# gkaissis/PriMIA

Measured on AMD Instinct MI355X. Metric: images_per_sec, higher is better.
Workload: dtype bf16; 1 GPU; ResNet-18 federated-client training step (fwd+loss+bwd+SGD), batch 256/client, 3x224x224, 1 client per GPU; batch_per_client=256, clients=1, sync_every_n_batch=3, dp_sgd=False

## Files before the change

### primia_amd/build.py

```python
import concurrent.futures
import os
import shutil
import subprocess
import sys

HERE = os.path.dirname(os.path.abspath(__file__))
CSRC = os.path.join(HERE, "csrc")
OBJ = os.path.join(CSRC, "_build")
ISA = os.path.join(OBJ, "isa")
LIB = os.path.join(HERE, "libprimia_hip.so")
ARCH = "gfx950"
FLAGS = ["-O3", "-std=c++17", "-fPIC", f"--offload-arch={ARCH}", "-Wno-unused-result"]


def source_digest(files=None):
    import hashlib

    names = sorted(f for f in os.listdir(CSRC) if f.endswith((".hip", ".h"))) if files is None else sorted(files)
    paths = [os.path.join(CSRC, f) for f in names]
    if files is None:
        paths.append(os.path.join(HERE, "..", "include", "primia_hip.h"))
    h = hashlib.sha256()
    for q in paths:
        h.update(os.path.basename(q).encode() + b"\0")
        import re

        text = re.sub(r"/\*.*?\*/", "", open(q, "r", encoding="utf-8", errors="replace").read(), flags=re.S)
        for line in text.splitlines():
            code = line.split("//", 1)[0].rstrip()
            if code:
                h.update(code.encode() + b"\n")
    return h.hexdigest()


def _hipcc():
    for c in ("/opt/rocm/bin/hipcc", "hipcc"):
        if os.path.isabs(c) and os.path.exists(c):
            return c
    return "hipcc"


def _newer(src, dst, deps=()):
    if not os.path.exists(dst):
        return True
    t = os.path.getmtime(dst)
    return any(os.path.getmtime(p) > t for p in (src, *deps))


def build(force=False, verbose=True):
    os.makedirs(OBJ, exist_ok=True)
    headers = [os.path.join(CSRC, f) for f in os.listdir(CSRC) if f.endswith(".h")]
    headers.append(os.path.join(HERE, "..", "include", "primia_hip.h"))
    sources = sorted(f for f in os.listdir(CSRC) if f.endswith(".hip"))
    jobs = []
    for f in sources:
        src = os.path.join(CSRC, f)
        obj = os.path.join(OBJ, f[:-4] + ".o")
        if force or _newer(src, obj, headers) or not os.path.exists(os.path.join(ISA, f[:-4] + ".s")):
            jobs.append((src, obj))

    def compile_one(job):
        src, obj = job
        name = os.path.basename(src)[:-4]
        tmp = os.path.join(OBJ, "tmp_" + name)
        shutil.rmtree(tmp, ignore_errors=True)
        os.makedirs(tmp)
        cmd = [_hipcc(), *FLAGS, "-save-temps=obj", "-c", src, "-o", os.path.join(tmp, name + ".o")]
        r = subprocess.run(cmd, capture_output=True, text=True)
        if r.returncode == 0:
            os.makedirs(ISA, exist_ok=True)
            os.replace(os.path.join(tmp, f"{name}-hip-amdgcn-amd-amdhsa-{ARCH}.s"), os.path.join(ISA, name + ".s"))
            os.replace(os.path.join(tmp, name + ".o"), obj)
        shutil.rmtree(tmp, ignore_errors=True)
        return src, r.returncode, r.stdout + r.stderr

    if jobs:
        with concurrent.futures.ThreadPoolExecutor(max_workers=min(6, len(jobs))) as ex:
            for src, rc, out in ex.map(compile_one, jobs):
                if verbose:
                    print(f"[primia build] {os.path.basename(src)}: {'ok' if rc == 0 else 'FAILED'}")
                if rc != 0:
                    raise RuntimeError(f"hipcc failed for {src}:\n{out}")
    objs = [os.path.join(OBJ, f[:-4] + ".o") for f in sources]
    if jobs or force or not os.path.exists(LIB):
        cmd = [_hipcc(), "-shared", "-fPIC", f"--offload-arch={ARCH}", "-o", LIB, *objs]
        r = subprocess.run(cmd, capture_output=True, text=True)
        if r.returncode != 0:
            raise RuntimeError("link failed:\n" + r.stdout + r.stderr)
        if verbose:
            print(f"[primia build] linked {LIB}")
    return LIB


PROBE_LIB = os.path.join(HERE, "..", "tools", "micro", "libprimia_probe.so")
PROBE_SOURCES = ("conv3x3_c64.hip", "conv_s2lh.hip", "options.hip")


def build_probe(extra_flags=()):
    build(verbose=False)
    objs = []
    for f in sorted(x for x in os.listdir(CSRC) if x.endswith(".hip")):
        if f in PROBE_SOURCES:
            os.makedirs(os.path.join(OBJ, "probe"), exist_ok=True)
            obj = os.path.join(OBJ, "probe", f[:-4] + ".o")
            cmd = [_hipcc(), *FLAGS, "-DPRIMIA_PROBE=1", *extra_flags, "-c", os.path.join(CSRC, f), "-o", obj]
            r = subprocess.run(cmd, capture_output=True, text=True)
            if r.returncode != 0:
                raise RuntimeError(f"hipcc failed for {f} (probe):\n{r.stdout}{r.stderr}")
        else:
            obj = os.path.join(OBJ, f[:-4] + ".o")
        objs.append(obj)
    r = subprocess.run([_hipcc(), "-shared", "-fPIC", f"--offload-arch={ARCH}", "-o", PROBE_LIB, *objs],
                       capture_output=True, text=True)
    if r.returncode != 0:
        raise RuntimeError("link failed:\n" + r.stdout + r.stderr)
    print(f"[primia build] linked {os.path.normpath(PROBE_LIB)}")
    return PROBE_LIB


if __name__ == "__main__":
    if "--probe" in sys.argv:
        build_probe()
    else:
        build(force="--force" in sys.argv)
```

### primia_amd/csrc/options.h

```cpp
#pragma once

namespace primia {

#define PRIMIA_OPTIONS(X)                                                                                              \
    X(lh2, 1)                                        \
    X(lh2_bm, 0)                                      \
    X(lh4, 1)                \
    X(c64_blocks, 512)                                         \
    X(c64_dbg, 0)                      \
    X(c64_stages, 4)                                                      \
    X(s2lh, 1)               \
    X(s2lh_dbg, 0)

enum OptId : int {
#define PRIMIA_OPT_ENUM(name, def) kOpt_##name,
    PRIMIA_OPTIONS(PRIMIA_OPT_ENUM)
#undef PRIMIA_OPT_ENUM
        kOptCount
};

extern int g_options[kOptCount];

inline int opt(OptId id) { return __atomic_load_n(&g_options[id], __ATOMIC_RELAXED); }

}

#define PRIMIA_OPT(name) (::primia::opt(::primia::kOpt_##name))
```

### primia_amd/csrc/options.hip

```cpp
#include <string.h>

#include <atomic>

#include "common.h"
#include "options.h"

#ifndef PRIMIA_PROBE
#define PRIMIA_PROBE 0
#endif

namespace primia {

int g_options[kOptCount] = {
#define PRIMIA_OPT_DEF(name, def) def,
    PRIMIA_OPTIONS(PRIMIA_OPT_DEF)
#undef PRIMIA_OPT_DEF
};

static const char* const kOptNames[kOptCount] = {
#define PRIMIA_OPT_NAME(name, def) #name,
    PRIMIA_OPTIONS(PRIMIA_OPT_NAME)
#undef PRIMIA_OPT_NAME
};

static const int kOptDefaults[kOptCount] = {
#define PRIMIA_OPT_DEF(name, def) def,
    PRIMIA_OPTIONS(PRIMIA_OPT_DEF)
#undef PRIMIA_OPT_DEF
};

static std::atomic<int64_t> g_options_epoch{0};

static int find_option(const char* name) {
    if (!name) return -1;
    for (int i = 0; i < kOptCount; ++i)
        if (!strcmp(name, kOptNames[i])) return i;
    return -1;
}

}

using namespace primia;

extern "C" {

int primia_set_option(const char* name, int value) {
    const int i = find_option(name);
    if (i < 0) return PRIMIA_ERR_ARG;
#if !PRIMIA_PROBE
    if ((i == kOpt_c64_dbg || i == kOpt_s2lh_dbg) && value != 0) return PRIMIA_ERR_UNSUPPORTED;
#endif
    if (__atomic_exchange_n(&g_options[i], value, __ATOMIC_RELAXED) != value)
        g_options_epoch.fetch_add(1, std::memory_order_release);
    return PRIMIA_OK;
}

int64_t primia_options_epoch(void) { return g_options_epoch.load(std::memory_order_acquire); }

int primia_get_option(const char* name, int* value) {
    const int i = find_option(name);
    if (i < 0 || !value) return PRIMIA_ERR_ARG;
    *value = __atomic_load_n(&g_options[i], __ATOMIC_RELAXED);
    return PRIMIA_OK;
}

int primia_reset_options(void) {
    bool moved = false;
    for (int i = 0; i < kOptCount; ++i) moved |= __atomic_exchange_n(&g_options[i], kOptDefaults[i], __ATOMIC_RELAXED) != kOptDefaults[i];
    if (moved) g_options_epoch.fetch_add(1, std::memory_order_release);
    return PRIMIA_OK;
}

int primia_option_count(void) { return kOptCount; }

int primia_option_name(int index, char* buf, int buf_len) {
    if (index < 0 || index >= kOptCount || !buf || buf_len <= (int)strlen(kOptNames[index])) return PRIMIA_ERR_ARG;
    strcpy(buf, kOptNames[index]);
    return PRIMIA_OK;
}

}
```

### primia_amd/csrc/stem_bwd_fused.hip

```cpp
#include <stdlib.h>

#include "conv_wgrad.h"

namespace primia {

__device__ __attribute__((aligned(16))) const unsigned char kStemFusedZeroPage[16] = {0};

__device__ __forceinline__ void sbf_dma16(const void* g, unsigned lds_addr) {
    asm volatile("s_mov_b32 m0, %1\n\ts_nop 0\n\tglobal_load_lds_dwordx4 %0, off" ::"v"(g), "s"(lds_addr) : "memory");
}

typedef int sbf_i32x4 __attribute__((ext_vector_type(4)));

__device__ __forceinline__ void sbf_bdma16(unsigned voff, sbf_i32x4 rsrc, unsigned lds_addr) {
    asm volatile("s_mov_b32 m0, %2\n\ts_nop 0\n\tbuffer_load_dwordx4 %0, %1, 0 offen lds"
                 ::"v"(voff), "s"(rsrc), "s"(lds_addr) : "memory");
}

__device__ __forceinline__ sbf_i32x4 sbf_rsrc(const void* base, long bytes) {
    const unsigned long long a = (unsigned long long)base;
    sbf_i32x4 r;
    r[0] = (int)(unsigned)a;
    r[1] = (int)(unsigned)(a >> 32) & 0xffff;
    r[2] = (int)(unsigned)(bytes > 0xfffffff0L ? 0xfffffff0L : bytes);
    r[3] = 0x00020000;
#pragma unroll
    for (int j = 0; j < 4; ++j) r[j] = __builtin_amdgcn_readfirstlane(r[j]);
    return r;
}
constexpr unsigned kSbfOob = 0xfffffff0u;

__device__ __forceinline__ int sbf_key(int slot) { return ((slot >> 1) & 1) | (((slot >> 3) & 1) << 1); }

__device__ __forceinline__ void sbf_wait_vmcnt(int n) {
    switch (n) {
        case 0: asm volatile("s_waitcnt vmcnt(0)" ::: "memory"); break;
        case 1: asm volatile("s_waitcnt vmcnt(1)" ::: "memory"); break;
        case 2: asm volatile("s_waitcnt vmcnt(2)" ::: "memory"); break;
        case 3: asm volatile("s_waitcnt vmcnt(3)" ::: "memory"); break;
        case 4: asm volatile("s_waitcnt vmcnt(4)" ::: "memory"); break;
        case 5: asm volatile("s_waitcnt vmcnt(5)" ::: "memory"); break;
        case 6: asm volatile("s_waitcnt vmcnt(6)" ::: "memory"); break;
        case 7: asm volatile("s_waitcnt vmcnt(7)" ::: "memory"); break;
        default: asm volatile("s_waitcnt vmcnt(8)" ::: "memory"); break;
    }
}

struct StemFusedParams {
    const bf16* xp;
    const bf16* y;
    const bf16* dpool;
    const uint8_t* argmax;
    const float *gamma, *beta, *mean, *invstd, *dbeta, *dgamma;
    float inv_m;
    float* dw;
    float* ws;
    int N, Hp, Wp, Ho, Wo, Hq, Wq;
    int PH, PW, PPI;
    int total, per_block;
    int debug;
};

constexpr int kSbfXB = 7 * 1024;
constexpr int kSbfTile = 16 * 1024;
constexpr int kSbfRaw = kSbfTile + 9 * 1024;
constexpr int kSbfRing = 5;
constexpr int kSbfRaw0 = 3 * kSbfXB;
constexpr int kSbfLds = kSbfRaw0 + kSbfRing * kSbfRaw;

__global__ __launch_bounds__(1024) void stem_bwd_fused_kernel(StemFusedParams p) {
    typedef __attribute__((address_space(3))) bf16x4_t* lds4_t;
    extern __shared__ __attribute__((aligned(16))) char smem[];
    const int tid = threadIdx.x, lane = tid & 63;
    const int wave = __builtin_amdgcn_readfirstlane(tid >> 6);
    const unsigned lds0 = (unsigned)(size_t)(__attribute__((address_space(3))) char*)smem;

    const int t0 = blockIdx.x * p.per_block;
    int t1 = t0 + p.per_block;
    if (t1 > p.total) t1 = p.total;
    const int n = t1 - t0;
    if (n <= 0) return;
    int cn = t0 / p.PPI, cph, cpw;
    {
        const int rem = t0 - cn * p.PPI;
        cph = rem / p.PW;
        cpw = rem - cph * p.PW;
    }
    auto advance = [&](int& an, int& aph, int& apw) {
        if (++apw == p.PW) {
            apw = 0;
            if (++aph == p.PH) {
                aph = 0;
                ++an;
            }
        }
    };

    if (wave >= 8) {
        const int tw = wave - 8;
        const int npc = tw == 0 ? 4 : 3;
        const sbf_i32x4 rs_y = sbf_rsrc(p.y, (long)p.N * p.Ho * p.Wo * 128);
        const sbf_i32x4 rs_g = sbf_rsrc(p.dpool, (long)p.N * p.Hq * p.Wq * 128);
        const sbf_i32x4 rs_c = sbf_rsrc(p.argmax, (long)p.N * p.Hq * p.Wq * 64);
        unsigned prel[4];
        int prow[4], pcol[4];
#pragma unroll
        for (int it = 0; it < 4; ++it) {
            const int idx = tw + 8 * it;
            prow[it] = pcol[it] = 0;
            if (idx < 16) {
                const int slot = idx * 8 + (lane >> 3), sl = lane & 7;
                const int chunk = ((((sl >> 1) ^ sbf_key(slot)) << 1) | (sl & 1));
                prel[it] = (unsigned)((((slot >> 4) * p.Wo + (slot & 15)) * 64 + chunk * 8) * 2);
            } else {
                const bool grad = idx < 22;
                const int G = (grad ? idx - 16 : idx - 22) * 64 + lane;
                const int slot = grad ? G >> 3 : G >> 2, sub = grad ? G & 7 : G & 3;
                const int row = slot / 9, col = slot - 9 * row;
                prow[it] = slot < 45 ? row : 1 << 20;
                pcol[it] = col;
                prel[it] = (unsigned)(grad ? (row * p.Wq + col) * 128 + sub * 16 : (row * p.Wq + col) * 64 + sub * 16);
            }
        }
        auto stage_raw = [&](int rbuf) {
            const unsigned ybase = (unsigned)(((cn * p.Ho + cph * 8) * p.Wo + cpw * 16) * 128);
            const int A0 = cph * 4, B0 = cpw * 8;
            const unsigned wpix = (unsigned)((cn * p.Hq + A0) * p.Wq + B0);
            const int rmax = p.Hq - A0, cmax = p.Wq - B0;
            advance(cn, cph, cpw);
#pragma unroll
            for (int it = 0; it < 4; ++it) {
                const int idx = tw + 8 * it;
                if (idx >= 25) break;
                const unsigned dst = __builtin_amdgcn_readfirstlane(lds0 + kSbfRaw0 + rbuf * kSbfRaw + idx * 1024);
                if (idx < 16) {
                    sbf_bdma16(prel[it] + ybase, rs_y, dst);
                } else {
                    const bool ok = prow[it] < rmax && pcol[it] < cmax;
                    if (idx < 22)
                        sbf_bdma16(ok ? prel[it] + wpix * 128u : kSbfOob, rs_g, dst);
                    else
                        sbf_bdma16(ok ? prel[it] + wpix * 64u : kSbfOob, rs_c, dst);
                }
            }
        };
        const int tt = tid - 512;
        const int c8 = tt & 7, bcol = (tt >> 3) & 7, brow = tw & 3, dg = tw >> 2;
        float k0[8], k1[8], k2[8], k3[8], k4[8], k5[8];
#pragma unroll
        for (int k = 0; k < 8; ++k) {
            const int c = c8 * 8 + k;
            const float is = p.invstd[c];
            k0[k] = p.mean[c];
            k1[k] = is;
            k2[k] = p.gamma[c] * is;
            k3[k] = p.dbeta[c] * p.inv_m;
            k4[k] = p.dgamma[c] * p.inv_m;
            k5[k] = p.beta[c];
        }
        __builtin_amdgcn_s_waitcnt(0x0f70);
        int tph = cph, tpw = cpw;
        typedef __attribute__((address_space(3))) char* ldsp_t;
        int offy[2];
#pragma unroll
        for (int r = 0; r < 2; ++r) {
            const int slot = (2 * brow + r) * 16 + 2 * bcol + (r ^ dg);
            offy[r] = slot * 128 + ((((c8 >> 1) ^ sbf_key(slot)) << 5) | ((c8 & 1) << 4));
        }
        const int offg = kSbfTile + (brow * 9 + bcol) * 128 + c8 * 16;
        const int offc = kSbfTile + 6 * 1024 + (brow * 9 + bcol) * 64 + c8 * 8;
        auto transform = [&](int rbuf) {
            const ldsp_t tile = (ldsp_t)(size_t)(lds0 + kSbfRaw0 + rbuf * kSbfRaw);
            const ldsp_t wg = tile + offg, wc = tile + offc;
            const bool rok = tph * 4 + brow + 1 < p.Hq, cok = tpw * 8 + bcol + 1 < p.Wq;
            if (++tpw == p.PW) {
                tpw = 0;
                if (++tph == p.PH) tph = 0;
            }
#pragma unroll
            for (int r = 0; r < 2; ++r) {
                const int j = r ^ dg;
                const ldsp_t yp = tile + offy[r];
                float vy[8], g[8];
                const u32x4 yraw = *(const __attribute__((address_space(3))) u32x4*)yp;
                Chunk<bf16>::unpack(yraw, vy);
#pragma unroll
                for (int k = 0; k < 8; ++k) g[k] = 0.f;
#pragma unroll
                for (int di = 1; di >= 0; --di) {
                    if (di > r) continue;
#pragma unroll
                    for (int dj = 1; dj >= 0; --dj) {
                        if (dj > j) continue;
                        const unsigned want = (unsigned)((1 + r - 2 * di) * 3 + (1 + j - 2 * dj));
                        const bool ok = (di == 0 || rok) && (dj == 0 || cok);
                        float wv[8];
                        const u32x4 wraw = *(const __attribute__((address_space(3))) u32x4*)(wg + (di * 9 + dj) * 128);
                        Chunk<bf16>::unpack(wraw, wv);
                        u32x2 codes = *(const __attribute__((address_space(3))) u32x2*)(wc + (di * 9 + dj) * 64);
                        if (!ok) codes = u32x2{0xffffffffu, 0xffffffffu};
#pragma unroll
                        for (int k = 0; k < 8; ++k)
                            g[k] += ((codes[k >> 2] >> (8 * (k & 3))) & 0xffu) == want ? wv[k] : 0.f;
                    }
                }
#pragma unroll
                for (int k = 0; k < 8; ++k) {
                    const float zz = __builtin_fmaf(vy[k] - k0[k], k2[k], k5[k]);
                    const float gi = zz > 0.f ? g[k] : 0.f;
                    const float xh = (vy[k] - k0[k]) * k1[k];
                    vy[k] = k2[k] * (gi - k3[k] - xh * k4[k]);
                }
                *(__attribute__((address_space(3))) u32x4*)yp = Chunk<bf16>::pack(vy);
            }
        };

        const bool raw_on = !(p.debug & 4);
        for (int s = 0; s < 3; ++s)
            if (s < n && raw_on) stage_raw(s);
        for (int k = -1; k < n; ++k) {
            const int inflight = (k + 2 < n ? npc : 0) + (k + 3 < n ? npc : 0);
            sbf_wait_vmcnt(raw_on ? inflight : 0);
            asm volatile("s_waitcnt lgkmcnt(0)" ::: "memory");
            __builtin_amdgcn_s_barrier();
            if (k + 4 < n && raw_on) stage_raw((k + 4) % kSbfRing);
            if (k + 1 < n && !(p.debug & 1)) transform((k + 1) % kSbfRing);
        }
        return;
    }

    const int kh = wave >> 2, rq = wave & 3;
    const int fr = lane & 15, fg = lane >> 4;
    const int tp = fr >> 2, tc8 = (fr & 3) * 8;
    const sbf_i32x4 rs_x = sbf_rsrc(p.xp, (long)p.N * p.Hp * p.Wp * 8);
    unsigned xrel;
    {
        const int G = wave * 64 + lane;
        const int row = G / 20, c16 = G - row * 20;
        xrel = G < 420 ? (unsigned)((row * p.Wp + 2 * c16) * 8) : kSbfOob;
    }
    auto stage_x = [&](int buf) {
        const unsigned xbase = (unsigned)(((cn * p.Hp + cph * 16) * p.Wp + cpw * 32) * 8);
        advance(cn, cph, cpw);
        if (wave < 7)
            sbf_bdma16(xrel == kSbfOob ? kSbfOob : xrel + xbase, rs_x,
                       __builtin_amdgcn_readfirstlane(lds0 + buf * kSbfXB + wave * 1024));
    };

    f32x4 acc[2][2][2];
#pragma unroll
    for (int i = 0; i < 2; ++i)
#pragma unroll
        for (int rr = 0; rr < 2; ++rr)
#pragma unroll
            for (int h = 0; h < 2; ++h) acc[i][rr][h] = f32x4{0.f, 0.f, 0.f, 0.f};

    typedef __attribute__((address_space(3))) char* ldsp_t;
    const int a_slot = 8 * fg + tp;
    int offa[2][2];
#pragma unroll
    for (int i = 0; i < 2; ++i)
#pragma unroll
        for (int h = 0; h < 2; ++h) {
            const int s0 = a_slot + 4 * h;
            offa[i][h] = s0 * 128 + (((2 * kh + i) ^ sbf_key(s0)) << 5) + tc8;
        }
    const int offb = ((fg >> 1) * 2) * 320 + 16 * (8 * (fg & 1) + tp) + tc8 + 2 * rq * 320;

    auto compute = [&](int xbuf, int rbuf) {
        const ldsp_t lb = (ldsp_t)(size_t)(lds0 + xbuf * kSbfXB) + offb;
        const ldsp_t la = (ldsp_t)(size_t)(lds0 + kSbfRaw0 + rbuf * kSbfRaw);
        ldsp_t pa[2][2];
#pragma unroll
        for (int i = 0; i < 2; ++i)
#pragma unroll
            for (int h = 0; h < 2; ++h) pa[i][h] = la + offa[i][h];
#pragma unroll
        for (int ks = 0; ks < 4; ++ks) {
            bf16x8_t a[2], b[2][2];
#pragma unroll
            for (int i = 0; i < 2; ++i) {
                bf16x4_t lo = __builtin_amdgcn_ds_read_tr16_b64_v4bf16((lds4_t)(pa[i][0] + ks * 4096));
                bf16x4_t hi = __builtin_amdgcn_ds_read_tr16_b64_v4bf16((lds4_t)(pa[i][1] + ks * 4096));
                a[i] = __builtin_shufflevector(lo, hi, 0, 1, 2, 3, 4, 5, 6, 7);
            }
#pragma unroll
            for (int rr = 0; rr < 2; ++rr) {
#pragma unroll
                for (int h = 0; h < 2; ++h) {
                    const ldsp_t q = lb + ((4 * ks + rr) * 320 + 32 * h);
                    bf16x4_t lo = __builtin_amdgcn_ds_read_tr16_b64_v4bf16((lds4_t)q);
                    bf16x4_t hi = __builtin_amdgcn_ds_read_tr16_b64_v4bf16((lds4_t)(q + 64));
                    b[rr][h] = __builtin_shufflevector(lo, hi, 0, 1, 2, 3, 4, 5, 6, 7);
                }
            }
#pragma unroll
            for (int rr = 0; rr < 2; ++rr) {
                if (2 * rq + rr == 7) continue;
#pragma unroll
                for (int h = 0; h < 2; ++h)
#pragma unroll
                    for (int i = 0; i < 2; ++i)
                        acc[i][rr][h] = __builtin_amdgcn_mfma_f32_16x16x32_bf16(a[i], b[rr][h], acc[i][rr][h], 0, 0, 0);
            }
        }
    };

    stage_x(0);
    if (n > 1) stage_x(1);
    for (int k = -1; k < n; ++k) {
        if (k + 1 < n && wave < 7)
            asm volatile("s_waitcnt vmcnt(1)" ::: "memory");
        else
            asm volatile("s_waitcnt vmcnt(0)" ::: "memory");
        __builtin_amdgcn_s_barrier();
        if (k < 0) continue;
        if (k + 2 < n) stage_x((k + 2) % 3);
        if (!(p.debug & 2)) compute(k % 3, k % kSbfRing);
    }

    if (p.ws) {
        float* o = p.ws + (long)blockIdx.x * (64 * 256);
#pragma unroll
        for (int rr = 0; rr < 2; ++rr) {
            const int r = 2 * rq + rr;
#pragma unroll
            for (int h = 0; h < 2; ++h) {
                const bool live = r < 7 && 16 * h + fr < 28;
#pragma unroll
                for (int i = 0; i < 2; ++i)
#pragma unroll
                    for (int j = 0; j < 4; ++j)
                        o[(32 * kh + 16 * i + 4 * fg + j) * 256 + r * 32 + 16 * h + fr] = live ? acc[i][rr][h][j] : 0.f;
            }
        }
        return;
    }
#pragma unroll
    for (int rr = 0; rr < 2; ++rr) {
        const int r = 2 * rq + rr;
        if (r == 7) continue;
#pragma unroll
        for (int h = 0; h < 2; ++h) {
            if (16 * h + fr >= 28) continue;
#pragma unroll
            for (int i = 0; i < 2; ++i)
#pragma unroll
                for (int j = 0; j < 4; ++j)
                    unsafeAtomicAdd(p.dw + (long)(32 * kh + 16 * i + 4 * fg + j) * 256 + r * 32 + 16 * h + fr, acc[i][rr][h][j]);
        }
    }
}

}

using namespace primia;

extern "C" int primia_stem_bwd_fused_ok(int N, int H, int W, int dtype) {
    if (dtype != PRIMIA_BF16 || N <= 0 || H <= 0 || W <= 0 || H % 32 != 0 || W % 32 != 0) return 0;
    if ((long)N * (H + 6) * (W + 8) * 4 >= (1L << 31) || (long)N * (H / 2) * (W / 2) * 64 >= (1L << 31)) return 0;
    int total, per_block, grid;
    return stem_wgrad_halo_blocks(N, H, W, &total, &per_block, &grid) ? 1 : 0;
}

extern "C" int primia_stem_bwd_fused(const void* x_padded, const void* y, const void* dpooled, const uint8_t* argmax,
                                     const float* gamma, const float* beta, const float* save_mean,
                                     const float* save_invstd, const float* dgamma, const float* dbeta, float* dw_acc,
                                     void* ws, int64_t ws_bytes, int N, int H, int W, int dtype,
                                     primia_stream_t stream) {
    PRIMIA_REQUIRE(x_padded && y && dpooled && argmax && gamma && beta && save_mean && save_invstd && dgamma && dbeta &&
                   dw_acc && N > 0 && H > 0 && W > 0);
    if (dtype != PRIMIA_BF16) return PRIMIA_ERR_UNSUPPORTED;
    if (H % 32 != 0 || W % 32 != 0) return PRIMIA_ERR_UNSUPPORTED;
    if ((long)N * (H + 6) * (W + 8) * 4 >= (1L << 31) || (long)N * (H / 2) * (W / 2) * 64 >= (1L << 31))
        return PRIMIA_ERR_UNSUPPORTED;
    StemFusedParams p;
    p.xp = (const bf16*)x_padded; p.y = (const bf16*)y; p.dpool = (const bf16*)dpooled; p.argmax = argmax;
    p.gamma = gamma; p.beta = beta; p.mean = save_mean; p.invstd = save_invstd; p.dbeta = dbeta; p.dgamma = dgamma;
    p.dw = dw_acc;
    p.N = N; p.Hp = H + 6; p.Wp = W + 8; p.Ho = H / 2; p.Wo = W / 2;
    p.Hq = (p.Ho + 2 - 3) / 2 + 1; p.Wq = (p.Wo + 2 - 3) / 2 + 1;
    p.inv_m = (float)(1.0 / ((double)N * p.Ho * p.Wo));
    p.PH = p.Ho / 8; p.PW = p.Wo / 16; p.PPI = p.PH * p.PW;
    int grid = 0;
    if (!stem_wgrad_halo_blocks(N, H, W, &p.total, &p.per_block, &grid)) return PRIMIA_ERR_UNSUPPORTED;
    const int64_t slab_bytes = (int64_t)grid * 64 * 256 * (int64_t)sizeof(float);
    const bool store = ws && ws_bytes >= slab_bytes;
    p.ws = store ? (float*)ws : nullptr;
    p.debug = 0;
    static bool attr_set = false;
    if (!attr_set) {
        if (hipFuncSetAttribute((const void*)stem_bwd_fused_kernel, hipFuncAttributeMaxDynamicSharedMemorySize, kSbfLds) !=
            hipSuccess)
            return PRIMIA_ERR_LAUNCH;
        attr_set = true;
    }
    hipStream_t st = (hipStream_t)stream;
    stem_bwd_fused_kernel<<<grid, 1024, kSbfLds, st>>>(p);
    if (store) wgrad_tile_reduce(p.ws, dw_acc, grid, 1, 64, 256, 1, 1, 4, 256, 1, st);
    return launch_status();
}
```

Baseline: 55460 images/s.

## Remap stem backward transform threads to 4-channel pixel slices with packed math

Restructures the transform warps of the fused stem backward kernel so each thread handles half of an 8-channel chunk across a 2x2 pixel quad, instead of 8 channels for two pixels. Weight loads and pool-argmax codes are hoisted and reused across the four output pixels. The compare-and-select selection now uses branchless bit masks over packed bf16, and the BN/ReLU backward math uses float2 packed FMA. It also routes the kernel's debug flags through a probe-only option so the debug branches compile away in production builds. The new thread mapping changes LDS access patterns and register usage, which could shift bank conflicts or occupancy.

```diff
diff --git a/primia_amd/build.py b/primia_amd/build.py
--- a/primia_amd/build.py
+++ b/primia_amd/build.py
@@ -93,7 +93,7 @@
 
 
 PROBE_LIB = os.path.join(HERE, "..", "tools", "micro", "libprimia_probe.so")
-PROBE_SOURCES = ("conv3x3_c64.hip", "conv_s2lh.hip", "options.hip")
+PROBE_SOURCES = ("conv3x3_c64.hip", "conv_s2lh.hip", "options.hip", "stem_bwd_fused.hip")
 
 
 def build_probe(extra_flags=()):
diff --git a/primia_amd/csrc/options.h b/primia_amd/csrc/options.h
--- a/primia_amd/csrc/options.h
+++ b/primia_amd/csrc/options.h
@@ -10,7 +10,8 @@
     X(c64_dbg, 0)                      \
     X(c64_stages, 4)                                                      \
     X(s2lh, 1)               \
-    X(s2lh_dbg, 0)
+    X(s2lh_dbg, 0)           \
+    X(stem_dbg, 0)
 
 enum OptId : int {
 #define PRIMIA_OPT_ENUM(name, def) kOpt_##name,
diff --git a/primia_amd/csrc/options.hip b/primia_amd/csrc/options.hip
--- a/primia_amd/csrc/options.hip
+++ b/primia_amd/csrc/options.hip
@@ -48,7 +48,7 @@
     const int i = find_option(name);
     if (i < 0) return PRIMIA_ERR_ARG;
 #if !PRIMIA_PROBE
-    if ((i == kOpt_c64_dbg || i == kOpt_s2lh_dbg) && value != 0) return PRIMIA_ERR_UNSUPPORTED;
+    if ((i == kOpt_c64_dbg || i == kOpt_s2lh_dbg || i == kOpt_stem_dbg) && value != 0) return PRIMIA_ERR_UNSUPPORTED;
 #endif
     if (__atomic_exchange_n(&g_options[i], value, __ATOMIC_RELAXED) != value)
         g_options_epoch.fetch_add(1, std::memory_order_release);
diff --git a/primia_amd/csrc/stem_bwd_fused.hip b/primia_amd/csrc/stem_bwd_fused.hip
--- a/primia_amd/csrc/stem_bwd_fused.hip
+++ b/primia_amd/csrc/stem_bwd_fused.hip
@@ -1,6 +1,11 @@
 #include <stdlib.h>
 
 #include "conv_wgrad.h"
+#include "options.h"
+
+#ifndef PRIMIA_PROBE
+#define PRIMIA_PROBE 0
+#endif
 
 namespace primia {
 
@@ -11,6 +16,8 @@
 }
 
 typedef int sbf_i32x4 __attribute__((ext_vector_type(4)));
+typedef float sbf_f32x2 __attribute__((ext_vector_type(2)));
+typedef __bf16 sbf_bf16x2 __attribute__((ext_vector_type(2)));
 
 __device__ __forceinline__ void sbf_bdma16(unsigned voff, sbf_i32x4 rsrc, unsigned lds_addr) {
     asm volatile("s_mov_b32 m0, %2\n\ts_nop 0\n\tbuffer_load_dwordx4 %0, %1, 0 offen lds"
@@ -80,6 +87,7 @@
     if (t1 > p.total) t1 = p.total;
     const int n = t1 - t0;
     if (n <= 0) return;
+    const int dbg = PRIMIA_PROBE ? p.debug : 0;
     int cn = t0 / p.PPI, cph, cpw;
     {
         const int rem = t0 - cn * p.PPI;
@@ -145,77 +153,88 @@
             }
         };
         const int tt = tid - 512;
-        const int c8 = tt & 7, bcol = (tt >> 3) & 7, brow = tw & 3, dg = tw >> 2;
-        float k0[8], k1[8], k2[8], k3[8], k4[8], k5[8];
-#pragma unroll
-        for (int k = 0; k < 8; ++k) {
-            const int c = c8 * 8 + k;
-            const float is = p.invstd[c];
-            k0[k] = p.mean[c];
-            k1[k] = is;
-            k2[k] = p.gamma[c] * is;
-            k3[k] = p.dbeta[c] * p.inv_m;
-            k4[k] = p.dgamma[c] * p.inv_m;
-            k5[k] = p.beta[c];
-        }
+        const int h = tt & 1, c8 = (tt >> 1) & 7, bcol = (tt >> 4) & 7, brow = tw >> 1;
+        sbf_f32x2 k0[2], k1[2], k2[2], k3[2], k4[2], k5[2];
+#pragma unroll
+        for (int q = 0; q < 2; ++q)
+#pragma unroll
+            for (int e = 0; e < 2; ++e) {
+                const int c = c8 * 8 + h * 4 + 2 * q + e;
+                const float is = p.invstd[c];
+                k0[q][e] = p.mean[c];
+                k1[q][e] = is;
+                k2[q][e] = p.gamma[c] * is;
+                k3[q][e] = p.dbeta[c] * p.inv_m;
+                k4[q][e] = p.dgamma[c] * p.inv_m;
+                k5[q][e] = p.beta[c];
+            }
         __builtin_amdgcn_s_waitcnt(0x0f70);
         int tph = cph, tpw = cpw;
         typedef __attribute__((address_space(3))) char* ldsp_t;
-        int offy[2];
-#pragma unroll
-        for (int r = 0; r < 2; ++r) {
-            const int slot = (2 * brow + r) * 16 + 2 * bcol + (r ^ dg);
-            offy[r] = slot * 128 + ((((c8 >> 1) ^ sbf_key(slot)) << 5) | ((c8 & 1) << 4));
-        }
-        const int offg = kSbfTile + (brow * 9 + bcol) * 128 + c8 * 16;
-        const int offc = kSbfTile + 6 * 1024 + (brow * 9 + bcol) * 64 + c8 * 8;
+        const int slot0 = brow * 32 + bcol * 2;
+        const int offy = slot0 * 128 + ((((c8 >> 1) ^ sbf_key(slot0)) << 5) | ((c8 & 1) << 4)) + h * 8;
+        const int offg = kSbfTile + (brow * 9 + bcol) * 128 + c8 * 16 + h * 8;
+        const int offc = kSbfTile + 6 * 1024 + (brow * 9 + bcol) * 64 + c8 * 8 + h * 4;
         auto transform = [&](int rbuf) {
             const ldsp_t tile = (ldsp_t)(size_t)(lds0 + kSbfRaw0 + rbuf * kSbfRaw);
-            const ldsp_t wg = tile + offg, wc = tile + offc;
+            const ldsp_t yp = tile + offy, wg = tile + offg, wc = tile + offc;
             const bool rok = tph * 4 + brow + 1 < p.Hq, cok = tpw * 8 + bcol + 1 < p.Wq;
             if (++tpw == p.PW) {
                 tpw = 0;
                 if (++tph == p.PH) tph = 0;
             }
-#pragma unroll
-            for (int r = 0; r < 2; ++r) {
-                const int j = r ^ dg;
-                const ldsp_t yp = tile + offy[r];
-                float vy[8], g[8];
-                const u32x4 yraw = *(const __attribute__((address_space(3))) u32x4*)yp;
-                Chunk<bf16>::unpack(yraw, vy);
-#pragma unroll
-                for (int k = 0; k < 8; ++k) g[k] = 0.f;
-#pragma unroll
-                for (int di = 1; di >= 0; --di) {
-                    if (di > r) continue;
-#pragma unroll
-                    for (int dj = 1; dj >= 0; --dj) {
-                        if (dj > j) continue;
-                        const unsigned want = (unsigned)((1 + r - 2 * di) * 3 + (1 + j - 2 * dj));
-                        const bool ok = (di == 0 || rok) && (dj == 0 || cok);
-                        float wv[8];
-                        const u32x4 wraw = *(const __attribute__((address_space(3))) u32x4*)(wg + (di * 9 + dj) * 128);
-                        Chunk<bf16>::unpack(wraw, wv);
-                        u32x2 codes = *(const __attribute__((address_space(3))) u32x2*)(wc + (di * 9 + dj) * 64);
-                        if (!ok) codes = u32x2{0xffffffffu, 0xffffffffu};
-#pragma unroll
-                        for (int k = 0; k < 8; ++k)
-                            g[k] += ((codes[k >> 2] >> (8 * (k & 3))) & 0xffu) == want ? wv[k] : 0.f;
+            unsigned wv[2][2][4], cs[2][2];
+#pragma unroll
+            for (int di = 0; di < 2; ++di)
+#pragma unroll
+                for (int dj = 0; dj < 2; ++dj) {
+                    const u32x2 wraw = *(const __attribute__((address_space(3))) u32x2*)(wg + (di * 9 + dj) * 128);
+                    const unsigned codes = *(const __attribute__((address_space(3))) unsigned*)(wc + (di * 9 + dj) * 64);
+#pragma unroll
+                    for (int q = 0; q < 2; ++q) {
+                        wv[di][dj][2 * q] = wraw[q] << 16;
+                        wv[di][dj][2 * q + 1] = wraw[q] & 0xffff0000u;
                     }
+                    const unsigned c7 = (codes & 0x7f7f7f7fu) | ((codes >> 1) & 0x40404040u);
+                    const bool ok = (di == 0 || rok) && (dj == 0 || cok);
+                    cs[di][dj] = ok ? c7 : 0x7f7f7f7fu;
                 }
 #pragma unroll
-                for (int k = 0; k < 8; ++k) {
-                    const float zz = __builtin_fmaf(vy[k] - k0[k], k2[k], k5[k]);
-                    const float gi = zz > 0.f ? g[k] : 0.f;
-                    const float xh = (vy[k] - k0[k]) * k1[k];
-                    vy[k] = k2[k] * (gi - k3[k] - xh * k4[k]);
+            for (int r = 0; r < 2; ++r)
+#pragma unroll
+                for (int j = 0; j < 2; ++j) {
+                    sbf_f32x2 g[2] = {sbf_f32x2{0.f, 0.f}, sbf_f32x2{0.f, 0.f}};
+#pragma unroll
+                    for (int di = r; di >= 0; --di)
+#pragma unroll
+                        for (int dj = j; dj >= 0; --dj) {
+                            const unsigned want = (unsigned)((1 + r - 2 * di) * 3 + (1 + j - 2 * dj));
+                            const unsigned m = (cs[di][dj] ^ ~(want * 0x01010101u)) + (0u - 0x7f7f7f7fu);
+#pragma unroll
+                            for (int q = 0; q < 2; ++q) {
+                                const unsigned lo = wv[di][dj][2 * q] & (unsigned)__builtin_amdgcn_sbfe((int)m, 16 * q + 7, 1);
+                                const unsigned hi = wv[di][dj][2 * q + 1] & (unsigned)__builtin_amdgcn_sbfe((int)m, 16 * q + 15, 1);
+                                g[q] += sbf_f32x2{__uint_as_float(lo), __uint_as_float(hi)};
+                            }
+                        }
+                    const ldsp_t yq = yp + r * 2048 + j * 128;
+                    const u32x2 yraw = *(const __attribute__((address_space(3))) u32x2*)yq;
+                    u32x2 o;
+#pragma unroll
+                    for (int q = 0; q < 2; ++q) {
+                        const sbf_f32x2 y2 = {__uint_as_float(yraw[q] << 16), __uint_as_float(yraw[q] & 0xffff0000u)};
+                        const sbf_f32x2 t2 = y2 - k0[q];
+                        const sbf_f32x2 zz = __builtin_elementwise_fma(t2, k2[q], k5[q]);
+                        const sbf_f32x2 gi = {zz[0] > 0.f ? g[q][0] : 0.f, zz[1] > 0.f ? g[q][1] : 0.f};
+                        const sbf_f32x2 xh = t2 * k1[q];
+                        const sbf_f32x2 d2 = k2[q] * (gi - k3[q] - xh * k4[q]);
+                        o[q] = __builtin_bit_cast(uint32_t, __builtin_convertvector(d2, sbf_bf16x2));
+                    }
+                    *(__attribute__((address_space(3))) u32x2*)yq = o;
                 }
-                *(__attribute__((address_space(3))) u32x4*)yp = Chunk<bf16>::pack(vy);
-            }
         };
 
-        const bool raw_on = !(p.debug & 4);
+        const bool raw_on = !(dbg & 4);
         for (int s = 0; s < 3; ++s)
             if (s < n && raw_on) stage_raw(s);
         for (int k = -1; k < n; ++k) {
@@ -224,7 +243,7 @@
             asm volatile("s_waitcnt lgkmcnt(0)" ::: "memory");
             __builtin_amdgcn_s_barrier();
             if (k + 4 < n && raw_on) stage_raw((k + 4) % kSbfRing);
-            if (k + 1 < n && !(p.debug & 1)) transform((k + 1) % kSbfRing);
+            if (k + 1 < n && !(dbg & 1)) transform((k + 1) % kSbfRing);
         }
         return;
     }
@@ -316,7 +335,7 @@
         __builtin_amdgcn_s_barrier();
         if (k < 0) continue;
         if (k + 2 < n) stage_x((k + 2) % 3);
-        if (!(p.debug & 2)) compute(k % 3, k % kSbfRing);
+        if (!(dbg & 2)) compute(k % 3, k % kSbfRing);
     }
 
     if (p.ws) {
@@ -387,7 +406,7 @@
     const int64_t slab_bytes = (int64_t)grid * 64 * 256 * (int64_t)sizeof(float);
     const bool store = ws && ws_bytes >= slab_bytes;
     p.ws = store ? (float*)ws : nullptr;
-    p.debug = 0;
+    p.debug = PRIMIA_PROBE ? PRIMIA_OPT(stem_dbg) : 0;
     static bool attr_set = false;
     if (!attr_set) {
         if (hipFuncSetAttribute((const void*)stem_bwd_fused_kernel, hipFuncAttributeMaxDynamicSharedMemorySize, kSbfLds) !=
```

Result: no change. 55420 images/s (-0.1%).
